# wjustin784/spMM

Hardware: AMD Instinct MI355X
Metric: CSR×CSR SpGEMM GFLOPS + peak HBM bytes, random N×N at stated density (higher is better)
Workload: dtype f64; 1 GPU; BASELINE config 4 (configs[3], ALG3 with its HBM cap): random CSR 65536x65536 density=0.005 float64 (spmm_amd.gen.random_csr on the device, seeds 42/43), ALG3, 1 chunk (cap not binding: the unchunked workspace is within chunk_fraction x P entries), chunk_fraction 0.2; N=65536, rows_per_rank=65536, alg=3, n_chunks=1, alg3_cap=not binding, nnzB=21465793, nnzA=21479711, nnzC=3460266668, num_products=7035505794, parallelism=single GPU

## Files before the change

spmm_amd/csrc/spgemm.hip:

```cpp
#include <hip/hip_runtime.h>
#include <hip/hip_ext.h>

#include <algorithm>
#include <atomic>
#include <cmath>
#include <cstdint>
#include <cstdio>
#include <cstdlib>
#include <cstring>
#include <limits>
#include <new>
#include <vector>

#include "spgemm.h"
#include "spgemm_kernels.hpp"
#include "spgemm_tile.hpp"
#include "spgemm_tile_dn.hpp"
#include "spgemm_spmv.hpp"
#include "spgemm_row.hpp"
#include "spgemm_spmm.hpp"
#include "spgemm_transpose.hpp"
#include "spgemm_geam.hpp"
#include "spgemm_canon.hpp"
#include "spgemm_extract.hpp"
#include "spgemm_dense.hpp"

using namespace spg;

constexpr int PINNED_WORDS = MIRROR_GEN_WORD + 1;

struct spg_handle_s {
    int device = 0;
    int cus = 256;
    hipStream_t stream = nullptr;
    int last_hip = 0;
    int64_t* pinned = nullptr;
    int64_t mirror_gen = 0;
    int32_t* spill_ctr = nullptr;
    bool spill_ctr_dirty = false;
    uint64_t lb_spin = SCAN_SPIN;
    bool lds_ordered = true;
    bool lds_ordered32 = true;
    void* scratch = nullptr;
    size_t scratch_bytes = 0;
    bool timing = false;
    struct Pending { int phase; hipEvent_t a, b; };
    std::vector<Pending> pending;
    std::vector<hipEvent_t> pool;
    double ms[SPG_NUM_PHASES] = {};
    int64_t launches[SPG_NUM_PHASES] = {};
    bool q_valid = false;
    spg_csr_t q_A{}, q_B{};
    spg_alg_t q_alg = SPG_ALG2;
    float q_cf = 0.f;
    int64_t q_P = -1, q_seg_len = 0;
    std::vector<int64_t> q_chunk_rows, q_chunk_nz;
};

struct spg_plan_s {
    spg_csr_t A{}, B{};
    spg_alg_t alg = SPG_ALG2;
    float cf = 0.2f;
    char* ws = nullptr;
    size_t ws_bytes = 0;
    int64_t* scalars = nullptr;
    int64_t* row_cnt = nullptr;
    uint32_t* seg = nullptr;
// ... 13 lines not shown
    bool lean = true;
    bool lean32 = true;
    int tws = 10;
    int G = 1;
    int rgs = 0;
    int twss = 10;
    bool sym_seg = false;
    bool sym_flags = false;
    bool counts_ready = false;
    unsigned long long* lb = nullptr;
    void* ext = nullptr;
    bool alg1_fused = false;
    bool fused_failed = false;
    bool scaled_in_place = false;
    int64_t sym_spills = -1;
    int64_t nspc = 0;
    int64_t* cspill = nullptr;
    std::vector<int64_t> chunk_spills;
    int64_t cap = 0;
    uint2* tidx = nullptr;
    int32_t* tptr = nullptr;
    bool packed = false;
    bool placed = false;
    uint2* pseg = nullptr;
    int32_t* segblk = nullptr;
    uint32_t* sidx = nullptr;
    void* brec = nullptr;
    uint16_t* bj16 = nullptr;
    bool brec_built = false;
    bool brec_cols = false;
    uint32_t* bitmap = nullptr;
    int64_t* item_cnt = nullptr;
    bool tidx_built = false;
    unsigned list_grid = 16;
    int symbolic_runs = 0;
    std::vector<int64_t> chunk_rows;
    std::vector<int64_t> chunk_nz;
};

namespace {

inline size_t align_up(size_t x, size_t a = 256) { return (x + a - 1) / a * a; }

inline size_t vbytes(spg_dtype_t t) {
    return t == SPG_C_64F ? 16 : (t == SPG_R_64F || t == SPG_C_32F) ? 8 : 4;
}

inline size_t brec_bytes(spg_dtype_t t) {
    return t == SPG_R_64F ? 10 : t == SPG_R_32F ? 6 : 4 + vbytes(t);
}

template <typename F>
spg_status_t dispatch_value(spg_dtype_t t, F&& f) {
    switch (t) {
#ifndef SPG_ONLY_F64
        case SPG_R_32F: return f(float(0));
        case SPG_C_32F: return f(cplx<float>(0));
        case SPG_C_64F: return f(cplx<double>(0));
#endif
        case SPG_R_64F: return f(double(0));
        default: break;
    }
    return SPG_STATUS_NOT_SUPPORTED;
}

template <typename F>
// ... 187 lines not shown
    return e;
}

struct PhaseTimer {
    spg_handle_t h;
    int phase;
    hipEvent_t a = nullptr;
    PhaseTimer(spg_handle_t h_, int phase_) : h(h_), phase(phase_) {
        if (h->timing && (a = take_event(h))) (void)hipEventRecord(a, h->stream);
    }
    ~PhaseTimer() {
        if (!a) return;
        hipEvent_t b = take_event(h);
        if (!b) { h->pool.push_back(a); return; }
        (void)hipEventRecord(b, h->stream);
        h->pending.push_back({phase, a, b});
    }
};

struct KernelTimer {
    spg_handle_t h;
    int phase;
    hipEvent_t a = nullptr, b = nullptr;
    KernelTimer(spg_handle_t h_, int phase_) : h(h_), phase(phase_) {
        if (!h->timing || !(a = take_event(h))) return;
        if (!(b = take_event(h))) { h->pool.push_back(a); a = nullptr; }
    }
    ~KernelTimer() {
        if (a && b) h->pending.push_back({phase, a, b});
    }
};

template <typename K, typename... Args>
inline void timed_launch(spg_handle_t h, int phase, K kernel, dim3 grid, dim3 block, Args... args) {
    KernelTimer kt(h, phase);
    hipExtLaunchKernelGGL(kernel, grid, block, 0, h->stream, kt.a, kt.b, 0, args...);
}

spg_status_t check_csr(const spg_csr_t* M) {
    if (!M) return SPG_STATUS_INVALID_VALUE;
    if (M->rows < 0 || M->cols < 0 || M->nnz < 0) return SPG_STATUS_INVALID_VALUE;
    if (M->cols > 2147483647LL) return SPG_STATUS_NOT_SUPPORTED;
    if (M->indptr_type != SPG_INDEX_32I && M->indptr_type != SPG_INDEX_64I)
        return SPG_STATUS_INVALID_VALUE;
    if (M->value_type != SPG_R_32F && M->value_type != SPG_R_64F && M->value_type != SPG_C_32F &&
        M->value_type != SPG_C_64F)
        return SPG_STATUS_NOT_SUPPORTED;
    if (M->indptr_type == SPG_INDEX_32I && M->nnz > 2147483647LL) return SPG_STATUS_INVALID_VALUE;
    if (!M->indptr && M->rows >= 0) return SPG_STATUS_INVALID_VALUE;
    if (M->nnz > 0 && (!M->indices || !M->values)) return SPG_STATUS_INVALID_VALUE;
    return SPG_STATUS_SUCCESS;
}

spg_status_t ensure_scratch(spg_handle_t h, size_t bytes) {
    if (h->scratch_bytes >= bytes) return SPG_STATUS_SUCCESS;
    if (h->scratch) {
        SPG_HIP(h, hipStreamSynchronize(h->stream));
        SPG_HIP(h, hipFree(h->scratch));
        h->scratch = nullptr;
        h->scratch_bytes = 0;
    }
    SPG_HIP(h, hipMalloc(&h->scratch, bytes));
    h->scratch_bytes = bytes;
    return SPG_STATUS_SUCCESS;
}

template <typename OUT, typename IN = int64_t>
spg_status_t launch_scan(spg_handle_t h, int64_t n, const IN* in, OUT* out,
                         unsigned long long* status, int64_t* scal, bool zero_status,
                         int32_t* move_cnt = nullptr, int64_t* move_dst = nullptr,
                         int64_t* host_mirror = nullptr, int64_t mirror_gen = 0, int mirror_n = 0,
                         const int64_t* seed = nullptr) {
    const int64_t tiles = scan_tiles(n);
    if (zero_status) SPG_HIP(h, hipMemsetAsync(status, 0, status_bytes(n), h->stream));
    timed_launch(h, SPG_PHASE_SCAN, k_scan_lb<OUT, IN>, dim3((unsigned)tiles), dim3(BLOCK), n, in, out, status, scal,
                 move_cnt, move_dst, host_mirror, mirror_gen, mirror_n, seed, h->lb_spin);
    SPG_LAUNCHED(h);
    return SPG_STATUS_SUCCESS;
}

template <typename IP>
spg_status_t launch_products(spg_handle_t h, const spg_csr_t& A, const spg_csr_t& B,
                             int64_t* cnt, int64_t* pref, int64_t* scal,
                             unsigned long long* status, bool zero_status) {
    const int64_t rows = A.rows;
    if (rows > 0) {
        PhaseTimer pt(h, SPG_PHASE_PRODUCTS);
        hipLaunchKernelGGL(k_row_products<IP>, dim3((unsigned)grid_for(rows, WPB)), dim3(BLOCK), 0,
                           h->stream, rows, (const IP*)A.indptr, (const int32_t*)A.indices,
                           (const IP*)B.indptr, cnt);
        SPG_LAUNCHED(h);
    }
    return launch_scan<int64_t>(h, rows, cnt, pref, status, scal, zero_status);
}

spg_status_t products_prefix(spg_handle_t h, const spg_csr_t& A, const spg_csr_t& B,
                             int64_t* cnt, int64_t* pref, int64_t* scal,
                             unsigned long long* status, bool zero_status = true) {
    return dispatch_index(A.indptr_type, [&](auto ip) {
        return launch_products<decltype(ip)>(h, A, B, cnt, pref, scal, status, zero_status);
    });
}

spg_status_t read_scalars(spg_handle_t h, const int64_t* dev, int n, int64_t* out);

spg_status_t products_total(spg_handle_t h, const spg_csr_t& A, const spg_csr_t& B, int64_t* P) {
    spg_status_t st = ensure_scratch(h, 256);
    if (st) return st;
    unsigned long long* acc = (unsigned long long*)h->scratch;
    SPG_HIP(h, hipMemsetAsync(acc, 0, sizeof(unsigned long long), h->stream));
    if (A.nnz > 0) {
// ... 84 lines not shown
    return e && std::strcmp(e, "1") == 0;
}
inline int64_t tile_item_slots(const spg_plan_s& p) { return tile_dense(p) ? p.A.rows * p.G : tile_items(p); }
inline int64_t* tile_chunk_items(const spg_plan_s& p, int64_t c) {
    return tile_dense(p) ? p.item_cnt + tile_chunk_r0(p, c) * p.G : p.item_cnt;
}
inline int sym_tiles(const spg_plan_s& p) { const int R = 1 << (p.twss - p.tws); return (p.G + R - 1) / R; }
inline int64_t rec_groups(const spg_plan_s& p) { return ((int64_t)p.G + (1 << p.rgs) - 1) >> p.rgs; }
inline int64_t tiles_padded(const spg_plan_s& p) { return rec_groups(p) << p.rgs; }
inline int64_t group_words(const spg_plan_s& p) { return (p.B.rows << p.rgs) + 1; }
inline int64_t bt_entries(const spg_plan_s& p) { return p.use_tile ? rec_groups(p) * group_words(p) : 0; }
constexpr double F32_RUN_MIN = 48;
inline bool fp32_runs(const spg_plan_s& p) {
    if (!p.lean32 || p.A.value_type != SPG_R_32F || p.B.cols <= 0 || p.B.rows <= 0 || (1 << p.tws) > 1024) return false;
    const char* e = std::getenv("SPG_F32_RUNS");
    if (e && std::strcmp(e, "0") == 0) return false;
    const double seg = (double)p.B.nnz / (double)p.B.rows * (double)(1 << p.tws) / (double)p.B.cols;
    return seg >= F32_RUN_MIN;
}
inline bool packed_segments(const spg_plan_s& p) {
    if (!tile_dense(p)) return false;
    if (p.A.value_type == SPG_R_32F) return fp32_runs(p);
    return p.lean && (p.A.value_type == SPG_R_64F || p.A.value_type == SPG_C_64F);
}
constexpr double SEG_PLACE_MIN_PRODUCTS = 4.0e9;
inline bool placed_segments(const spg_plan_s& p) {
    if (!packed_segments(p) || p.B.rows <= 0 || p.B.cols <= 0) return false;
    const char* e = std::getenv("SPG_SEG_PLACE");
    if (e && (std::strcmp(e, "1") == 0 || std::strcmp(e, "0") == 0)) return e[0] == '1';
    const double avgB = (double)p.B.nnz / (double)p.B.rows;
    const double seg = avgB * (double)(1 << p.tws) / (double)p.B.cols;
    return seg * (double)brec_bytes(p.A.value_type) <= (double)SEG_PLACE_MAX &&
           (double)p.A.nnz * avgB >= SEG_PLACE_MIN_PRODUCTS;
}
inline int64_t seg_blocks(const spg_plan_s& p) { return p.placed ? (int64_t)p.G * grid_for(p.B.rows, SEG_BLK) : 0; }
inline size_t brec_span(const spg_plan_s& p) {
    const size_t rb = brec_bytes(p.A.value_type);
    if (!p.placed) return rb * (size_t)p.B.nnz;
    return align_up((size_t)seg_bound((uint64_t)p.B.nnz, (uint64_t)p.B.rows * (uint64_t)p.G, (uint32_t)rb), SEG_LINE);
}
constexpr int SP_RGS = 3;
inline int record_group_log2(const spg_plan_s& p) {
    if (!p.use_tile || tile_dense(p) || !p.lean) return 0;
    if (p.A.value_type != SPG_R_64F || p.tws != 13) return 0;
    const char* e = std::getenv("SPG_SP_RECORD_GROUP");
    if (e && std::strcmp(e, "1") == 0) return 0;
    return SP_RGS;
}

inline bool fused_alg1(const spg_plan_s& p) {
    return p.alg == SPG_ALG1 && p.use_short && !p.use_tile && p.A.rows <= (1LL << 24);
}
inline bool alg1_upper_bound(const spg_plan_s& p) { return p.alg == SPG_ALG1 && !p.use_tile && !fused_alg1(p); }

inline size_t status_words(const spg_plan_s& p) {
    return 2 * (size_t)(scan_tiles(p.A.rows) + 1) +
           (p.use_tile ? (size_t)scan_tiles(tile_items(p)) + 1 + (size_t)scan_tiles(bt_entries(p)) + 1 : 0) +
           (p.placed ? (size_t)scan_tiles(seg_blocks(p)) + 1 : 0) +
           (fused_alg1(p) ? (size_t)std::max<int64_t>(grid_for(p.A.rows, ShortSmall::WPB), row_groups(p.A.rows)) + 1 : 0);
}
inline unsigned long long* rowptr_scan_status(const spg_plan_s& p) { return p.scan_status + scan_tiles(p.A.rows) + 1; }
inline unsigned long long* item_scan_status(const spg_plan_s& p) {
    return p.scan_status + 2 * (scan_tiles(p.A.rows) + 1);
}
inline unsigned long long* bt_scan_status(const spg_plan_s& p) {
    return item_scan_status(p) + scan_tiles(tile_items(p)) + 1;
// ... 232 lines not shown
                                   (RowExt<IP>*)nullptr, RowScan<OFF>{});
            else
                hipLaunchKernelGGL((k_short<T, IP, OFF, MODE, ShortSmall>), dim3((unsigned)grid_for(n, ShortSmall::WPB)),
                                   dim3(ShortSmall::WPB * WAVE), 0, h->stream, r0, n, p.B.cols, Ap, Aj, Ax, Bp, Bj,
                                   Bx, off, cj, cx, alpha, p.row_cnt, l1, cnt, (const int32_t*)nullptr,
                                   (const int32_t*)nullptr, (unsigned long long*)nullptr, (OFF*)nullptr,
                                   (int64_t*)nullptr, (int64_t)0);
            SPG_LAUNCHED(h);
        }
        if (p.sym_spills == 0) return SPG_STATUS_SUCCESS;
        PhaseTimer ps(h, SPG_PHASE_SPILL);
        hipLaunchKernelGGL((k_numeric<T, IP, OFF, UB>), dim3(p.list_grid), dim3(BLOCK), 0, h->stream,
                           r0, n, p.B.cols, Ap, Aj, Ax, Bp, Bj, Bx, off, cj, cx, alpha, p.row_cnt,
                           p.seg, nz0, p.seg_len, (const int32_t*)l1, (const int32_t*)cnt);
    } else {
        PhaseTimer pt(h, SPG_PHASE_NUMERIC);
        hipLaunchKernelGGL((k_numeric<T, IP, OFF, UB>), dim3((unsigned)grid_for(n, WPB)), dim3(BLOCK), 0,
                           h->stream, r0, n, p.B.cols, Ap, Aj, Ax, Bp, Bj, Bx, off, cj, cx, alpha,
                           p.row_cnt, p.seg, nz0, p.seg_len, (const int32_t*)nullptr,
                           (const int32_t*)nullptr);
    }
    SPG_LAUNCHED(h);
    return SPG_STATUS_SUCCESS;
}

template <typename OUT>
spg_status_t run_scan(spg_handle_t h, spg_plan_s& p, void* out, int mirror_n = 0) {
    return launch_scan<OUT>(h, p.A.rows, (const int64_t*)p.row_cnt, (OUT*)out,
                            rowptr_scan_status(p), p.scalars, false, nullptr, nullptr,
                            mirror_n ? h->pinned : nullptr, mirror_n ? ++h->mirror_gen : 0, mirror_n);
}

template <typename IP>
spg_status_t tile_build_index(spg_handle_t h, spg_plan_s& p) {
    if (p.tidx_built) return SPG_STATUS_SUCCESS;
    const IP* Bp = (const IP*)p.B.indptr;
    const int32_t* Bj = (const int32_t*)p.B.indices;
    const int R = 1 << (p.twss - p.tws);
    {
        const int Gp = (int)tiles_padded(p);
        timed_launch(h, SPG_PHASE_LAYOUT, k_tile_index<IP>, dim3((unsigned)grid_for(p.B.rows, 4)), dim3(256), p.B.rows,
                     Bp, Bj, p.tws, Gp, p.tidx);
        SPG_LAUNCHED(h);
        const int64_t n2 = p.B.rows * Gp + rec_groups(p);
        timed_launch(h, SPG_PHASE_LAYOUT, k_bt_count,
                     dim3((unsigned)std::max<int64_t>(1, std::min<int64_t>(grid_for(n2, 256), 65536))), dim3(256),
                     p.B.rows, Gp, p.G, R, (const uint2*)p.tidx, p.tptr, p.sidx, p.rgs);
        SPG_LAUNCHED(h);
        timed_launch(h, SPG_PHASE_LAYOUT, k_bj16,
                     dim3((unsigned)std::max<int64_t>(1, std::min<int64_t>(grid_for(p.B.nnz, 256), 65536))), dim3(256),
                     p.B.nnz, Bj, p.bj16);
        SPG_LAUNCHED(h);
    }
    spg_status_t st = launch_scan<int32_t, int32_t>(h, bt_entries(p), p.tptr, p.tptr, bt_scan_status(p),
                                                    p.scalars + 2, false);
    if (st) return st;
    if (p.placed) {
        const int64_t nblk = seg_blocks(p);
        const dim3 grid((unsigned)std::max<int64_t>(1, grid_for(nblk, 256)));
        const uint32_t rb = (uint32_t)brec_bytes(p.A.value_type);
        timed_launch(h, SPG_PHASE_LAYOUT, k_seg_place<false>, grid, dim3(256), p.B.rows, p.G, rb,
                     (const int32_t*)p.tptr, p.segblk, p.pseg, (char*)p.brec);
        SPG_LAUNCHED(h);
        if ((st = launch_scan<int32_t, int32_t>(h, nblk, p.segblk, p.segblk, seg_scan_status(p), p.scalars + 6, false)))
            return st;
        timed_launch(h, SPG_PHASE_LAYOUT, k_seg_place<true>, grid, dim3(256), p.B.rows, p.G, rb,
                     (const int32_t*)p.tptr, p.segblk, p.pseg, (char*)p.brec);
        SPG_LAUNCHED(h);
    }
    p.tidx_built = true;
    return SPG_STATUS_SUCCESS;
}

template <typename IP>
spg_status_t tile_sym_chunk(spg_handle_t h, spg_plan_s& p, int64_t c) {
    const int64_t r0 = tile_chunk_r0(p, c), n = tile_chunk_r1(p, c) - r0;
    int64_t* items = tile_chunk_items(p, c);
    if (n > 0) {
        if (p.sym_flags) {
            constexpr int W = SYM_FLAG_W;
            KernelTimer kt(h, SPG_PHASE_SYMBOLIC);
            hipExtLaunchKernelGGL((k_tile_sym_flag<IP, W>), dim3(coop_grid(n * sym_tiles(p), W)), dim3(W * WAVE),
                                  (size_t)1 << p.twss, h->stream, kt.a, kt.b, 0, r0, n, p.tws, p.G, p.twss,
                                  (const IP*)p.A.indptr, (const int32_t*)p.A.indices, (const IP*)p.B.indptr,
                                  (const uint16_t*)p.bj16, (const uint32_t*)p.sidx, items);
        } else if (p.sym_seg) {
            timed_launch(h, SPG_PHASE_SYMBOLIC, k_tile_sym_seg<IP>, dim3(tile_grid(n * sym_tiles(p), SEG_WPB)),
                         dim3(SEG_WPB * WAVE), r0, n, p.tws, p.G, p.twss, (const IP*)p.A.indptr,
                         (const int32_t*)p.A.indices, (const IP*)p.B.indptr, (const uint16_t*)p.bj16,
                         (const uint32_t*)p.sidx, tile_dense(p) ? (uint32_t*)nullptr : p.bitmap, items,
                         sym_full(p) ? p.B.cols : (int64_t)0);
        } else {
            timed_launch(h, SPG_PHASE_SYMBOLIC, k_tile_sym8c<IP, SYM8_CW>,
                         dim3(coop_grid(n * sym_tiles(p), SYM8_CW)), dim3(SYM8_CW * WAVE),
                         r0, n, p.tws, p.G, p.twss, (const IP*)p.A.indptr, (const int32_t*)p.A.indices,
                         (const IP*)p.B.indptr, (const uint16_t*)p.bj16, (const uint32_t*)p.sidx,
                         tile_dense(p) ? (uint32_t*)nullptr : p.bitmap, items);
        }
        SPG_LAUNCHED(h);
    }
    const int64_t nch = tile_chunks(p);
    int64_t* scal = c == nch - 1 ? p.scalars : p.scalars + 12 + 2 * (c & 1);
    const int64_t* seed = c == 0 ? nullptr : p.scalars + 12 + 2 * ((c - 1) & 1);
    return launch_scan<int64_t>(h, n * p.G, (const int64_t*)items, items, item_scan_status(p), scal,
                                true, nullptr, nullptr, nullptr, 0, 0, seed);
}

template <typename OUT>
spg_status_t tile_rowptr_chunk(spg_handle_t h, spg_plan_s& p, int64_t c, void* cp) {
    const int64_t r0 = tile_chunk_r0(p, c), n = tile_chunk_r1(p, c) - r0;
    timed_launch(h, SPG_PHASE_SCAN, k_items_to_rowptr<OUT>, dim3((unsigned)grid_for(n + 1, 256)), dim3(256), n, p.G,
                 (const int64_t*)tile_chunk_items(p, c), (OUT*)cp + r0);
    SPG_LAUNCHED(h);
    return SPG_STATUS_SUCCESS;
}

template <typename IP, typename OUT>
spg_status_t tile_symbolic(spg_handle_t h, spg_plan_s& p, void* cp) {
    spg_status_t st;
    if ((st = tile_build_index<IP>(h, p))) return st;
    const int64_t nch = tile_chunks(p);
    if ((nch == 1 || tile_dense(p)) && p.counts_ready) {
        for (int64_t c = 0; c < nch; ++c)
            if ((st = tile_rowptr_chunk<OUT>(h, p, c, cp))) return st;
        return SPG_STATUS_SUCCESS;
    }
    for (int64_t c = 0; c < nch; ++c) {
        if ((st = tile_sym_chunk<IP>(h, p, c))) return st;
        if ((st = tile_rowptr_chunk<OUT>(h, p, c, cp))) return st;
    }
    return SPG_STATUS_SUCCESS;
}

template <typename T, typename IP>
spg_status_t tile_numeric(spg_handle_t h, spg_plan_s& p, int32_t* cj, T* cx, T alpha, int64_t g0 = 0,
                          int64_t g1 = -1, const T* tm = nullptr) {
    if (g1 < 0) g1 = p.G;
    const IP* Ap = (const IP*)p.A.indptr;
    const IP* Bp = (const IP*)p.B.indptr;
    const int32_t* Aj = (const int32_t*)p.A.indices;
    const int32_t* Bj = (const int32_t*)p.B.indices;
    const T* Ax = (const T*)p.A.values;
    const T* Bx = (const T*)p.B.values;
    if (tm) {
        if (!p.brec_cols) {
            timed_launch(h, SPG_PHASE_LAYOUT, k_bt_pack<T, IP, 1>, dim3((unsigned)grid_for(p.B.rows, 4)), dim3(256),
                         p.B.rows, Bp, Bj, Bx, p.tws, (const int32_t*)p.tptr, (uint32_t*)p.brec, p.B.nnz, (T*)nullptr,
                         p.rgs, p.pseg, seg_end(p), seg_pairs(p), p.G);
            SPG_LAUNCHED(h);
            p.brec_cols = true;
        }
        p.brec_built = false;
        const int32_t* tp = (const int32_t*)p.tptr;
        const int64_t W = group_words(p);
        const int64_t q0 = g0 >> p.rgs, q1 = (g1 + (1 << p.rgs) - 1) >> p.rgs;
        const int64_t est = std::max<int64_t>(1, p.B.nnz * (q1 - q0) / std::max<int64_t>(rec_groups(p), 1));
        if (p.placed)
            timed_launch(h, SPG_PHASE_LAYOUT, k_bt_fill_pk<T>,
                         dim3((unsigned)std::max<int64_t>(1, std::min<int64_t>(grid_for((q1 - q0) * grid_for(p.B.rows, WAVE), 4), 16384))),
                         dim3(256), p.B.rows, q0, q1, tp, (const uint2*)p.pseg, tm, (uint32_t*)p.brec);
        else
            timed_launch(h, SPG_PHASE_LAYOUT, k_bt_fill<T>,
                         dim3((unsigned)std::max<int64_t>(1, std::min<int64_t>(grid_for(est, 256), 16384))), dim3(256),
                         tp + q0 * W, tp + (q1 - 1) * W + (W - 1), tm, (uint32_t*)p.brec);
        SPG_LAUNCHED(h);
    } else if (!p.brec_built) {
        timed_launch(h, SPG_PHASE_LAYOUT, k_bt_pack<T, IP>, dim3((unsigned)grid_for(p.B.rows, 4)), dim3(256), p.B.rows,
                     Bp, Bj, Bx, p.tws, (const int32_t*)p.tptr, (uint32_t*)p.brec, p.B.nnz, (T*)nullptr, p.rgs,
                     p.pseg, seg_end(p), seg_pairs(p), p.G);
        SPG_LAUNCHED(h);
        p.brec_built = true;
        p.brec_cols = true;
    }
    auto sent = [&](int r) {
        return (uint32_t)(((uint64_t)(p.packed ? 0 : p.B.nnz) + (uint64_t)r * SENT_N) * (uint64_t)rec_bytes<T>());
    };
    const int64_t nch = tile_chunks(p);
    for (int64_t c = 0; c < nch; ++c) {
        spg_status_t st;
        if (nch > 1 && !tile_dense(p) && (st = tile_sym_chunk<IP>(h, p, c))) return st;
        const int64_t r0 = tile_chunk_r0(p, c), n = tile_chunk_r1(p, c) - r0;
        if (n <= 0) continue;
        uint32_t it_lo = (uint32_t)(g0 * n), it_hi = (uint32_t)(g1 * n);
        int64_t nit = (g1 - g0) * n;
        KernelTimer kt(h, SPG_PHASE_NUMERIC);
        const bool dense = tile_dense(p);
        auto launch = [&](auto dn) {
            constexpr bool DN = decltype(dn)::value;
            constexpr int WPBN = tile_num_wpb<DN>();
            hipExtLaunchKernelGGL((k_tile<T, IP, DN>), dim3(tile_grid(nit, WPBN)), dim3(WPBN * WAVE), 0,
                                  h->stream, kt.a, kt.b, 0, r0, n, p.tws, p.G, Ap, Aj, Ax, p.B.rows,
                                  (const uint32_t*)p.brec, (const int32_t*)p.tptr,
                                  dense ? (const uint32_t*)nullptr : (const uint32_t*)p.bitmap,
                                  (const int64_t*)tile_chunk_items(p, c), cj, cx, alpha, it_lo, it_hi, p.rgs);
        };
        if constexpr (std::is_same<T, float>::value) {
            if (dense && p.packed) {
                hipExtLaunchKernelGGL((k_tile_dn<T, IP, 1024>), dim3(tile_grid(nit, DN_WPB)), dim3(DN_WPB * WAVE),
                                      0, h->stream, kt.a, kt.b, 0, r0, n, p.tws, p.G, Ap, Aj, Ax, p.B.rows,
                                      (const uint32_t*)p.brec, (const uint2*)p.pseg, (const int32_t*)seg_end(p),
                                      (const int64_t*)tile_chunk_items(p, c), cj, cx, alpha,
                                      sent(sentinel_region(1024)), it_lo, it_hi);
                SPG_LAUNCHED(h);
                continue;
            }
// ... 231 lines not shown
spg_status_t symbolic_rows(spg_handle_t h, spg_plan_s& p, void* cp, spg_index_t ct, int64_t* nnzC);

spg_status_t symbolic_alg1_short(spg_handle_t h, spg_plan_s& p, void* cp, spg_index_t ct, int64_t* nnzC) {
    spg_status_t st;
    ++p.symbolic_runs;
    if (p.counts_ready) {
        SPG_HIP(h, hipMemsetAsync(rowptr_scan_status(p), 0, status_bytes(p.A.rows), h->stream));
        if ((st = dispatch_index(ct, [&](auto out) { return run_scan<decltype(out)>(h, p, cp); }))) return st;
        int64_t tot;
        if ((st = read_scalars(h, p.scalars, 1, &tot))) return st;
        if (past_int32(ct, tot)) return SPG_STATUS_OVERFLOW;
        return symbolic_done(p, cp, ct, tot, nnzC);
    }
    st = dispatch_value(p.A.value_type, [&](auto tag) {
        return dispatch_index(p.A.indptr_type, ct, [&](auto ip, auto out) {
            return alg1_short_launch<decltype(tag), decltype(ip), decltype(out)>(h, p, cp);
        });
    });
    if (st) return st;
    int64_t sc[11];
    if ((st = read_scalars(h, p.scalars, 11, sc))) return st;
    if (sc[LB_FAIL] || sc[LB_CAPX]) {
        p.fused_failed = true;
        p.symbolic_runs = 0;
        return symbolic_rows(h, p, cp, ct, nnzC);
    }
    p.counts_ready = true;
    p.alg1_fused = true;
    if (past_int32(ct, sc[LB_TOTAL])) return SPG_STATUS_OVERFLOW;
    return symbolic_done(p, cp, ct, sc[LB_TOTAL], nnzC);
}

spg_status_t symbolic_tiles(spg_handle_t h, spg_plan_s& p, void* cp, spg_index_t ct, int64_t* nnzC) {
    spg_status_t st = dispatch_index(p.A.indptr_type, ct, [&](auto ip, auto out) {
        return tile_symbolic<decltype(ip), decltype(out)>(h, p, cp);
    });
    if (st) return st;
    int64_t tot;
    if ((st = read_scalars(h, p.scalars, 1, &tot))) return st;
    p.counts_ready = true;
    if (past_int32(ct, tot)) return SPG_STATUS_OVERFLOW;
    return symbolic_done(p, cp, ct, tot, nnzC);
}

spg_status_t symbolic_rows(spg_handle_t h, spg_plan_s& p, void* cp, spg_index_t ct, int64_t* nnzC) {
    spg_status_t st;
    if (p.symbolic_runs++ > 0) {
        SPG_HIP(h, hipMemsetAsync(rowptr_scan_status(p), 0, status_bytes(p.A.rows), h->stream));
    }
    const bool counted = !p.counts_ready;
    if (counted) {
        if (alg1_upper_bound(p)) {
            st = dispatch_value(p.A.value_type, [&](auto tag) {
                using T = decltype(tag);
                return dispatch_index(p.A.indptr_type, [&](auto ip) {
                    return run_numeric_rows<T, decltype(ip), int64_t, true>(h, p, 0, p.A.rows, 0, p.ub, p.tj,
                                                                            (T*)p.tx, (T)1);
                });
            });
        } else {
            st = dispatch_index(p.A.indptr_type, [&](auto ip) { return symbolic_typed<decltype(ip)>(h, p); });
        }
        if (st) return st;
    }
    const bool chunks = p.nspc > 0 && counted;
    const int nread = chunks ? 16 + p.nspc : 5;
    if ((st = dispatch_index(ct, [&](auto out) { return run_scan<decltype(out)>(h, p, cp, nread); }))) return st;
    std::vector<int64_t> all((size_t)nread);
    if ((st = wait_mirror(h))) return st;
    for (int i = 0; i < nread; ++i) all[(size_t)i] = ((volatile int64_t*)h->pinned)[i];
    if (chunks) {
        p.chunk_spills.assign(all.begin() + 16, all.end());
// ... 730 lines not shown
        case SPG_STATUS_HIP_ERROR: return "SPG_STATUS_HIP_ERROR";
    }
    return "SPG_STATUS_UNKNOWN";
}

spg_status_t spg_create(spg_handle_t* handle, int hip_device) {
    if (!handle) return SPG_STATUS_INVALID_VALUE;
    *handle = nullptr;
    int ndev = 0;
    if (hipGetDeviceCount(&ndev) != hipSuccess || ndev <= 0) return SPG_STATUS_NOT_INITIALIZED;
    int dev = hip_device;
    if (dev < 0) {
        if (hipGetDevice(&dev) != hipSuccess) return SPG_STATUS_NOT_INITIALIZED;
    }
    if (dev >= ndev) return SPG_STATUS_INVALID_VALUE;
    hipDeviceProp_t prop;
    if (hipGetDeviceProperties(&prop, dev) != hipSuccess) return SPG_STATUS_NOT_INITIALIZED;
    if (std::strncmp(prop.gcnArchName, "gfx950", 6) != 0) return SPG_STATUS_ARCH_MISMATCH;
    spg_handle_s* h = new (std::nothrow) spg_handle_s();
    if (!h) return SPG_STATUS_ALLOC_FAILED;
    h->device = dev;
    h->cus = prop.multiProcessorCount > 0 ? prop.multiProcessorCount : 256;
    if (const char* e = std::getenv("SPG_LB_SPIN_TICKS")) h->lb_spin = std::strtoull(e, nullptr, 10);
    DeviceGuard dg_(dev);
    hipError_t e = dg_.err;
    if (e == hipSuccess) e = lds_order_check(&h->lds_ordered, &h->lds_ordered32);
    if (const char* o = std::getenv("SPG_LDS_ORDERED"))
        if (std::strcmp(o, "0") == 0) h->lds_ordered = h->lds_ordered32 = false;
    if (e == hipSuccess)
        e = hipHostMalloc((void**)&h->pinned, PINNED_WORDS * sizeof(int64_t), hipHostMallocCoherent | hipHostMallocMapped);
    if (e == hipSuccess) std::memset(h->pinned, 0, PINNED_WORDS * sizeof(int64_t));
    if (e == hipSuccess) e = hipMalloc((void**)&h->spill_ctr, 256);
    if (e == hipSuccess) e = hipMemset(h->spill_ctr, 0, 256);
    if (e != hipSuccess) {
        delete h;
        return e == hipErrorOutOfMemory ? SPG_STATUS_ALLOC_FAILED : SPG_STATUS_HIP_ERROR;
    }
    *handle = h;
    return SPG_STATUS_SUCCESS;
}

spg_status_t spg_destroy(spg_handle_t h) {
    if (!h) return SPG_STATUS_NOT_INITIALIZED;
    (void)hipStreamSynchronize(h->stream);
    if (h->scratch) (void)hipFree(h->scratch);
    if (h->pinned) (void)hipHostFree(h->pinned);
    if (h->spill_ctr) (void)hipFree(h->spill_ctr);
    for (auto& q : h->pending) { (void)hipEventDestroy(q.a); (void)hipEventDestroy(q.b); }
    for (hipEvent_t e : h->pool) (void)hipEventDestroy(e);
    delete h;
    return SPG_STATUS_SUCCESS;
}

spg_status_t spg_set_stream(spg_handle_t h, void* stream) {
    if (!h) return SPG_STATUS_NOT_INITIALIZED;
    if ((hipStream_t)stream != h->stream) SPG_HIP(h, hipStreamSynchronize(h->stream));
    h->stream = (hipStream_t)stream;
    return SPG_STATUS_SUCCESS;
}

int spg_last_hip_error(spg_handle_t h) { return h ? h->last_hip : 0; }

spg_status_t spg_plan(spg_handle_t h, const spg_csr_t* A, const spg_csr_t* B, spg_alg_t alg,
                      float chunk_fraction, size_t* workspace_bytes, void* workspace,
                      spg_plan_t* plan) {
    if (!h) return SPG_STATUS_NOT_INITIALIZED;
    if (!workspace_bytes) return SPG_STATUS_INVALID_VALUE;
    spg_status_t st;
    if ((st = check_csr(A)) || (st = check_csr(B))) return st;
    if (A->cols != B->rows) return SPG_STATUS_INVALID_VALUE;
    if (A->value_type != B->value_type) return SPG_STATUS_INVALID_VALUE;
    if (A->indptr_type != B->indptr_type) return SPG_STATUS_INVALID_VALUE;
    if (alg != SPG_ALG_DEFAULT && alg != SPG_ALG1 && alg != SPG_ALG2 && alg != SPG_ALG3)
        return SPG_STATUS_INVALID_VALUE;
    if (alg == SPG_ALG3 && !(chunk_fraction > 0.0f && chunk_fraction <= 1.0f))
        return SPG_STATUS_INVALID_VALUE;
    if (workspace && !plan) return SPG_STATUS_INVALID_VALUE;
    DeviceGuard dg_(h->device);
    SPG_HIP(h, dg_.err);

    spg_plan_s tmp;
    tmp.A = *A;
    tmp.B = *B;
    tmp.alg = alg == SPG_ALG_DEFAULT ? SPG_ALG2 : alg;
    tmp.cf = chunk_fraction;
    tmp.seg_len = A->nnz;
    tmp.use_short = want_short(*A, *B);
    tmp.use_row = row_kernel_enabled();
    tmp.lean = h->lds_ordered;
    tmp.lean32 = h->lds_ordered32;
    tmp.use_tile = !tmp.use_short && want_tile(*A, *B, tmp.tws, tmp.G, tmp.lean);
    if (tmp.use_tile) {
        tmp.twss = sym_tile_log2(*B, tmp.tws, &tmp.sym_seg);
        tmp.rgs = record_group_log2(tmp);
        tmp.packed = packed_segments(tmp);
        tmp.placed = placed_segments(tmp);
        tmp.sym_flags = want_sym_flags(tmp);
    }
    tmp.list_grid = (unsigned)std::max<int64_t>(1, std::min<int64_t>(256, grid_for(A->rows, 64)));
    const bool same_as_query = h->q_valid && h->q_alg == tmp.alg && h->q_cf == chunk_fraction &&
                               std::memcmp(&h->q_A, A, sizeof(spg_csr_t)) == 0 &&
                               std::memcmp(&h->q_B, B, sizeof(spg_csr_t)) == 0;
    if (fused_alg1(tmp)) {
        const double avgB = B->rows > 0 ? (double)B->nnz / (double)B->rows : 0.0;
        const double est = 1.15 * (double)A->nnz * avgB + 4096.0;
        const double full = (double)A->rows * (double)B->cols;
        tmp.cap = (int64_t)std::min(est, full);
    } else if (alg1_upper_bound(tmp)) {
        if (workspace && same_as_query) {
            tmp.P = h->q_P;
        } else if ((st = products_total(h, *A, *B, &tmp.P))) {
            return st;
        }
    } else if (tmp.alg == SPG_ALG3) {
        if (workspace && same_as_query) {
            tmp.P = h->q_P;
            tmp.chunk_rows = h->q_chunk_rows;
            tmp.chunk_nz = h->q_chunk_nz;
            tmp.seg_len = h->q_seg_len;
        } else {
            spg_plan_s whole = tmp;
            whole.chunk_rows.assign({0, A->rows});
            whole.chunk_nz.assign({0, A->nnz});
            whole.seg_len = tmp.use_tile ? 1 : A->nnz;
            const char* ae = std::getenv("SPG_ALG3_CHUNK_ALWAYS");
            const bool always = ae && std::strcmp(ae, "1") == 0;
            if ((st = products_total(h, *A, *B, &tmp.P))) return st;
            const double cap = (double)chunk_fraction * (double)std::max<int64_t>(tmp.P, 0) *
                               (double)(sizeof(int32_t) + vbytes(A->value_type));
            if (always || (double)make_layout(whole).total > cap) {
// ... 572 lines not shown
    if (!p || !info || capacity < 0 || (capacity > 0 && !chunk_rows)) return SPG_STATUS_INVALID_VALUE;
    info->path = p->use_tile ? 2 : (p->use_short ? 1 : 0);
    info->tile_width = p->use_tile ? (1 << p->tws) : 0;
    info->tiles_per_row = p->use_tile ? p->G : 0;
    info->record_group = p->use_tile ? (1 << p->rgs) : 0;
    info->dense_tiles = tile_dense(*p) ? 1 : 0;
    const bool chunked = p->alg == SPG_ALG3 && p->chunk_rows.size() > 1;
    info->n_chunks = chunked ? (int64_t)p->chunk_rows.size() - 1 : 1;
    info->lds_ordered = p->use_tile && p->lean && (p->A.value_type == SPG_R_64F || p->A.value_type == SPG_C_64F) ? 1 : 0;
    if (tile_dense(*p) && fp32_runs(*p)) info->lds_ordered = 1;
    for (int64_t i = 0; i < std::min<int64_t>(capacity, info->n_chunks + 1); ++i)
        chunk_rows[i] = chunked ? p->chunk_rows[(size_t)i] : (i == 0 ? 0 : p->A.rows);
    return SPG_STATUS_SUCCESS;
}

spg_status_t spg_plan_destroy(spg_plan_t p) {
    if (!p) return SPG_STATUS_INVALID_VALUE;
    delete p;
    return SPG_STATUS_SUCCESS;
}

spg_status_t spg_spgemm_ws(spg_handle_t h, const spg_csr_t* A, const spg_csr_t* B, spg_alg_t alg,
                           float chunk_fraction, const void* alpha, void* workspace, size_t workspace_bytes,
                           void* C_indptr, spg_index_t C_indptr_type, int64_t* nnzC, void** C_indices,
                           void** C_values, size_t* peak_bytes, spg_plan_t* plan_out) {
    if (!h) return SPG_STATUS_NOT_INITIALIZED;
    if (!alpha || !nnzC || !C_indices || !C_values || !peak_bytes || !plan_out) return SPG_STATUS_INVALID_VALUE;
    *plan_out = nullptr;
    *C_indices = *C_values = nullptr;
    spg_plan_t p = nullptr;
    size_t wsb = workspace_bytes;
    spg_status_t st = spg_plan(h, A, B, alg, chunk_fraction, &wsb, workspace, &p);
    if (st) return st;
    if ((st = spg_symbolic(h, p, C_indptr, C_indptr_type, nnzC))) {
        spg_plan_destroy(p);
        return st;
    }
    const size_t ipc = C_indptr_type == SPG_INDEX_32I ? 4 : 8;
    if (p->alg1_fused && *nnzC > 0) {
        spg_csr_t C{p->A.rows, p->B.cols, *nnzC, C_indptr, p->tj, p->tx, C_indptr_type, p->A.value_type};
        st = spg_numeric(h, p, alpha, &C);
        if (!st) {
            *C_indices = p->tj;
            *C_values = p->tx;
            *peak_bytes = p->ws_bytes + ipc * (size_t)(p->A.rows + 1);
        }
        spg_plan_destroy(p);
        return st;
    }
    *peak_bytes = p->ws_bytes + ipc * (size_t)(p->A.rows + 1) +
                  (size_t)*nnzC * (sizeof(int32_t) + vbytes(p->A.value_type));
    *plan_out = p;
    return SPG_STATUS_SUCCESS;
}

spg_status_t spg_set_timing(spg_handle_t h, int enable) {
    if (!h) return SPG_STATUS_NOT_INITIALIZED;
    SPG_HIP(h, hipStreamSynchronize(h->stream));
    for (auto& q : h->pending) { h->pool.push_back(q.a); h->pool.push_back(q.b); }
    h->pending.clear();
    for (int i = 0; i < SPG_NUM_PHASES; ++i) { h->ms[i] = 0.0; h->launches[i] = 0; }
    h->timing = enable != 0;
    return SPG_STATUS_SUCCESS;
}

spg_status_t spg_get_timing(spg_handle_t h, spg_timing_t* t) {
// ... 18 lines not shown
```

spmm_amd/cusparse.py:

```python
from __future__ import annotations

import ctypes
from dataclasses import dataclass

import numpy as np
import torch

from . import _fastpath, _lib
from ._lib import SpgCsr, SpgError, check
from .sparse import csr_matrix

_VT = {torch.float32: _lib.SPG_R_32F, torch.float64: _lib.SPG_R_64F,
       torch.complex64: _lib.SPG_C_32F, torch.complex128: _lib.SPG_C_64F}
_ALPHA_CT = {torch.float32: (ctypes.c_float, 1), torch.float64: (ctypes.c_double, 1),
             torch.complex64: (ctypes.c_float, 2), torch.complex128: (ctypes.c_double, 2)}
_IT = {torch.int32: _lib.SPG_INDEX_32I, torch.int64: _lib.SPG_INDEX_64I}
_ALG = {1: _lib.SPG_ALG1, 2: _lib.SPG_ALG2, 3: _lib.SPG_ALG3}


@dataclass
class SpgemmStats:
    alg: int = 0
    workspace_bytes: int = 0
    peak_bytes: int = 0
# ... 132 lines not shown
    if before_numeric is not None and algo == _lib.SPG_ALG1:
        before_numeric()
        before_numeric = None
    if by_tiles is not None and algo == _lib.SPG_ALG1:
        if by_tiles(None) is not None:
            raise RuntimeError("by_tiles must complete B's values when geom is None")
        by_tiles = None
    if by_tiles is not None:
        return _spgemm_by_tiles(h, a, b, alpha, algo, cf, by_tiles, verbose, values_first)
    if fp is not None:
        al = complex(alpha)
        st, data, indices, indptr, wsb, peak = fp.spgemm(
            h.ptr.value, m, a.shape[1], n, a.indptr, a.indices, a.data, b.indptr, b.indices, b.data,
            int(algo), cf, al.real, al.imag)
        check(st, "spg_spgemm_ws")
        if verbose:
            print("USING ALG", alg, "workspace GB =", wsb / (1024 ** 3))
        last_stats.alg, last_stats.workspace_bytes = int(algo), int(wsb)
        last_stats.peak_bytes, last_stats.nnz = int(peak), int(indices.numel())
        return csr_matrix._from_parts(data, indices, indptr, (m, n), canonical=True)
    lib = h.lib
    va, vb = _csr_view(a), _csr_view(b)
    ws_bytes = ctypes.c_size_t(0)
    check(lib.spg_plan(h.ptr, ctypes.byref(va), ctypes.byref(vb), algo, cf,
                       ctypes.byref(ws_bytes), None, None), "spg_plan")
    if verbose:
        print("USING ALG", alg, "workspace GB =", ws_bytes.value / (1024 ** 3))
    ws = torch.empty(max(ws_bytes.value, 1), dtype=torch.uint8, device=dev)
    ct, nparts = _ALPHA_CT[a.data.dtype]
    al = (ct * 2)(complex(alpha).real, complex(alpha).imag) if nparts == 2 else ct(float(alpha))
    nnz, peak = ctypes.c_int64(0), ctypes.c_size_t(0)
    pj, px, plan = ctypes.c_void_p(), ctypes.c_void_p(), ctypes.c_void_p()
    wide = a.nnz * (b.nnz / max(b.shape[0], 1)) >= 2 ** 31
    for it in ((torch.int64,) if wide else (torch.int32, torch.int64)):
        indptr = torch.empty(m + 1, dtype=it, device=dev)
        st = lib.spg_spgemm_ws(h.ptr, ctypes.byref(va), ctypes.byref(vb), algo, cf, ctypes.byref(al),
                               ctypes.c_void_p(ws.data_ptr()), ws_bytes.value,
                               ctypes.c_void_p(indptr.data_ptr()), _IT[it], ctypes.byref(nnz),
                               ctypes.byref(pj), ctypes.byref(px), ctypes.byref(peak), ctypes.byref(plan))
        if st != _lib.STATUS_OVERFLOW:
            break
    check(st, "spg_spgemm_ws")
    nnzc = int(nnz.value)
    if pj.value:
        base = ws.data_ptr()
        oj, ox = pj.value - base, px.value - base
        indices = ws[oj:oj + 4 * nnzc].view(torch.int32)
        data = ws[ox:ox + a.data.element_size() * nnzc].view(a.data.dtype)
    else:
        try:
            indices = torch.empty(nnzc, dtype=torch.int32, device=dev)
            data = torch.empty(nnzc, dtype=a.data.dtype, device=dev)
            vc = SpgCsr(m, n, nnzc, indptr.data_ptr(), indices.data_ptr() if nnzc else 0,
                        data.data_ptr() if nnzc else 0, _IT[indptr.dtype], _VT[data.dtype])
            if before_numeric is not None:
                before_numeric()
            check(lib.spg_numeric(h.ptr, plan, ctypes.byref(al), ctypes.byref(vc)), "spg_numeric")
        finally:
            lib.spg_plan_destroy(plan)
    if wide and nnzc < 2 ** 31:
        indptr = indptr.to(torch.int32)
    last_stats.alg, last_stats.workspace_bytes = int(algo), int(ws_bytes.value)
    last_stats.peak_bytes, last_stats.nnz = int(peak.value), nnzc
    return csr_matrix._from_parts(data, indices, indptr, (m, n), canonical=True)


def _alpha_of(dtype, alpha):
    ct, nparts = _ALPHA_CT[dtype]
    return (ct * 2)(complex(alpha).real, complex(alpha).imag) if nparts == 2 else ct(float(alpha))


def _spgemm_by_tiles(h, a, b, alpha, algo, cf, by_tiles, verbose, values_first=True):
    lib = h.lib
    m, n = a.shape[0], b.shape[1]
    dev = a.device
# ... 682 lines not shown
```

Before: 695.3 GFLOPS.

## Overlap tile layout scan and record packing with symbolic phase on side stream

Splits the B tile-index build into a head (index, count, bj16) on the main stream and a tail (scan, segment placement, and optionally early record packing) run on a new side stream forked by event. The symbolic row-pointer chunks run concurrently on the main stream, and the main stream waits on a join event afterwards. When the chunks are mirrored, the symbolic total is read through a pinned host mirror instead of a device readback. The Python path also changes to call plan/symbolic separately when before_numeric is set. The cost is extra stream/event management, and any ordering mistake between the streams would be a hazard.

Measured after the change: 675.7 GFLOPS. 0.972x the previous value.

```diff
diff --git a/spmm_amd/csrc/spgemm.hip b/spmm_amd/csrc/spgemm.hip
--- a/spmm_amd/csrc/spgemm.hip
+++ b/spmm_amd/csrc/spgemm.hip
@@ -33,6 +33,8 @@
     int device = 0;
     int cus = 256;
     hipStream_t stream = nullptr;
+    hipStream_t side = nullptr;
+    hipEvent_t ev_fork = nullptr, ev_join = nullptr;
     int last_hip = 0;
     int64_t* pinned = nullptr;
     int64_t mirror_gen = 0;
@@ -112,6 +114,8 @@
     uint32_t* bitmap = nullptr;
     int64_t* item_cnt = nullptr;
     bool tidx_built = false;
+    bool overlap = true;
+    bool pack_early = false;
     unsigned list_grid = 16;
     int symbolic_runs = 0;
     std::vector<int64_t> chunk_rows;
@@ -365,9 +369,14 @@
 };
 
 template <typename K, typename... Args>
+inline void timed_launch_on(spg_handle_t h, hipStream_t stream, int phase, K kernel, dim3 grid, dim3 block,
+                            Args... args) {
+    KernelTimer kt(h, phase);
+    hipExtLaunchKernelGGL(kernel, grid, block, 0, stream, kt.a, kt.b, 0, args...);
+}
+template <typename K, typename... Args>
 inline void timed_launch(spg_handle_t h, int phase, K kernel, dim3 grid, dim3 block, Args... args) {
-    KernelTimer kt(h, phase);
-    hipExtLaunchKernelGGL(kernel, grid, block, 0, h->stream, kt.a, kt.b, 0, args...);
+    timed_launch_on(h, h->stream, phase, kernel, grid, block, args...);
 }
 
 spg_status_t check_csr(const spg_csr_t* M) {
@@ -399,17 +408,26 @@
 }
 
 template <typename OUT, typename IN = int64_t>
+spg_status_t launch_scan_on(spg_handle_t h, hipStream_t stream, int64_t n, const IN* in, OUT* out,
+                            unsigned long long* status, int64_t* scal, bool zero_status,
+                            int32_t* move_cnt = nullptr, int64_t* move_dst = nullptr,
+                            int64_t* host_mirror = nullptr, int64_t mirror_gen = 0, int mirror_n = 0,
+                            const int64_t* seed = nullptr) {
+    const int64_t tiles = scan_tiles(n);
+    if (zero_status) SPG_HIP(h, hipMemsetAsync(status, 0, status_bytes(n), stream));
+    timed_launch_on(h, stream, SPG_PHASE_SCAN, k_scan_lb<OUT, IN>, dim3((unsigned)tiles), dim3(BLOCK), n, in, out,
+                    status, scal, move_cnt, move_dst, host_mirror, mirror_gen, mirror_n, seed, h->lb_spin);
+    SPG_LAUNCHED(h);
+    return SPG_STATUS_SUCCESS;
+}
+template <typename OUT, typename IN = int64_t>
 spg_status_t launch_scan(spg_handle_t h, int64_t n, const IN* in, OUT* out,
                          unsigned long long* status, int64_t* scal, bool zero_status,
                          int32_t* move_cnt = nullptr, int64_t* move_dst = nullptr,
                          int64_t* host_mirror = nullptr, int64_t mirror_gen = 0, int mirror_n = 0,
                          const int64_t* seed = nullptr) {
-    const int64_t tiles = scan_tiles(n);
-    if (zero_status) SPG_HIP(h, hipMemsetAsync(status, 0, status_bytes(n), h->stream));
-    timed_launch(h, SPG_PHASE_SCAN, k_scan_lb<OUT, IN>, dim3((unsigned)tiles), dim3(BLOCK), n, in, out, status, scal,
-                 move_cnt, move_dst, host_mirror, mirror_gen, mirror_n, seed, h->lb_spin);
-    SPG_LAUNCHED(h);
-    return SPG_STATUS_SUCCESS;
+    return launch_scan_on<OUT, IN>(h, h->stream, n, in, out, status, scal, zero_status, move_cnt, move_dst,
+                                   host_mirror, mirror_gen, mirror_n, seed);
 }
 
 template <typename IP>
@@ -560,6 +578,10 @@
     const double seg = avgB * (double)(1 << p.tws) / (double)p.B.cols;
     return seg * (double)brec_bytes(p.A.value_type) <= (double)SEG_PLACE_MAX &&
            (double)p.A.nnz * avgB >= SEG_PLACE_MIN_PRODUCTS;
+}
+inline bool layout_overlap() {
+    const char* e = std::getenv("SPG_LAYOUT_OVERLAP");
+    return !(e && std::strcmp(e, "0") == 0);
 }
 inline int64_t seg_blocks(const spg_plan_s& p) { return p.placed ? (int64_t)p.G * grid_for(p.B.rows, SEG_BLK) : 0; }
 inline size_t brec_span(const spg_plan_s& p) {
@@ -858,48 +880,70 @@
 }
 
 template <typename IP>
-spg_status_t tile_build_index(spg_handle_t h, spg_plan_s& p) {
-    if (p.tidx_built) return SPG_STATUS_SUCCESS;
+spg_status_t tile_index_head(spg_handle_t h, spg_plan_s& p) {
     const IP* Bp = (const IP*)p.B.indptr;
     const int32_t* Bj = (const int32_t*)p.B.indices;
     const int R = 1 << (p.twss - p.tws);
-    {
-        const int Gp = (int)tiles_padded(p);
-        timed_launch(h, SPG_PHASE_LAYOUT, k_tile_index<IP>, dim3((unsigned)grid_for(p.B.rows, 4)), dim3(256), p.B.rows,
-                     Bp, Bj, p.tws, Gp, p.tidx);
-        SPG_LAUNCHED(h);
-        const int64_t n2 = p.B.rows * Gp + rec_groups(p);
-        timed_launch(h, SPG_PHASE_LAYOUT, k_bt_count,
-                     dim3((unsigned)std::max<int64_t>(1, std::min<int64_t>(grid_for(n2, 256), 65536))), dim3(256),
-                     p.B.rows, Gp, p.G, R, (const uint2*)p.tidx, p.tptr, p.sidx, p.rgs);
-        SPG_LAUNCHED(h);
-        timed_launch(h, SPG_PHASE_LAYOUT, k_bj16,
-                     dim3((unsigned)std::max<int64_t>(1, std::min<int64_t>(grid_for(p.B.nnz, 256), 65536))), dim3(256),
-                     p.B.nnz, Bj, p.bj16);
-        SPG_LAUNCHED(h);
-    }
-    spg_status_t st = launch_scan<int32_t, int32_t>(h, bt_entries(p), p.tptr, p.tptr, bt_scan_status(p),
-                                                    p.scalars + 2, false);
+    const int Gp = (int)tiles_padded(p);
+    timed_launch(h, SPG_PHASE_LAYOUT, k_tile_index<IP>, dim3((unsigned)grid_for(p.B.rows, 4)), dim3(256), p.B.rows,
+                 Bp, Bj, p.tws, Gp, p.tidx);
+    SPG_LAUNCHED(h);
+    const int64_t n2 = p.B.rows * Gp + rec_groups(p);
+    timed_launch(h, SPG_PHASE_LAYOUT, k_bt_count,
+                 dim3((unsigned)std::max<int64_t>(1, std::min<int64_t>(grid_for(n2, 256), 65536))), dim3(256),
+                 p.B.rows, Gp, p.G, R, (const uint2*)p.tidx, p.tptr, p.sidx, p.rgs);
+    SPG_LAUNCHED(h);
+    timed_launch(h, SPG_PHASE_LAYOUT, k_bj16,
+                 dim3((unsigned)std::max<int64_t>(1, std::min<int64_t>(grid_for(p.B.nnz, 256), 65536))), dim3(256),
+                 p.B.nnz, Bj, p.bj16);
+    SPG_LAUNCHED(h);
+    return SPG_STATUS_SUCCESS;
+}
+
+inline spg_status_t tile_index_tail(spg_handle_t h, spg_plan_s& p, hipStream_t stream) {
+    spg_status_t st = launch_scan_on<int32_t, int32_t>(h, stream, bt_entries(p), p.tptr, p.tptr, bt_scan_status(p),
+                                                       p.scalars + 2, false);
     if (st) return st;
     if (p.placed) {
         const int64_t nblk = seg_blocks(p);
         const dim3 grid((unsigned)std::max<int64_t>(1, grid_for(nblk, 256)));
         const uint32_t rb = (uint32_t)brec_bytes(p.A.value_type);
-        timed_launch(h, SPG_PHASE_LAYOUT, k_seg_place<false>, grid, dim3(256), p.B.rows, p.G, rb,
-                     (const int32_t*)p.tptr, p.segblk, p.pseg, (char*)p.brec);
+        timed_launch_on(h, stream, SPG_PHASE_LAYOUT, k_seg_place<false>, grid, dim3(256), p.B.rows, p.G, rb,
+                        (const int32_t*)p.tptr, p.segblk, p.pseg, (char*)p.brec);
         SPG_LAUNCHED(h);
-        if ((st = launch_scan<int32_t, int32_t>(h, nblk, p.segblk, p.segblk, seg_scan_status(p), p.scalars + 6, false)))
+        if ((st = launch_scan_on<int32_t, int32_t>(h, stream, nblk, p.segblk, p.segblk, seg_scan_status(p),
+                                                   p.scalars + 6, false)))
             return st;
-        timed_launch(h, SPG_PHASE_LAYOUT, k_seg_place<true>, grid, dim3(256), p.B.rows, p.G, rb,
-                     (const int32_t*)p.tptr, p.segblk, p.pseg, (char*)p.brec);
+        timed_launch_on(h, stream, SPG_PHASE_LAYOUT, k_seg_place<true>, grid, dim3(256), p.B.rows, p.G, rb,
+                        (const int32_t*)p.tptr, p.segblk, p.pseg, (char*)p.brec);
         SPG_LAUNCHED(h);
     }
+    return SPG_STATUS_SUCCESS;
+}
+
+template <typename IP>
+spg_status_t tile_build_index(spg_handle_t h, spg_plan_s& p) {
+    if (p.tidx_built) return SPG_STATUS_SUCCESS;
+    spg_status_t st;
+    if ((st = tile_index_head<IP>(h, p)) || (st = tile_index_tail(h, p, h->stream))) return st;
     p.tidx_built = true;
     return SPG_STATUS_SUCCESS;
 }
 
+template <typename T, typename IP>
+spg_status_t tile_pack_records(spg_handle_t h, spg_plan_s& p, hipStream_t stream) {
+    timed_launch_on(h, stream, SPG_PHASE_LAYOUT, k_bt_pack<T, IP>, dim3((unsigned)grid_for(p.B.rows, 4)), dim3(256),
+                    p.B.rows, (const IP*)p.B.indptr, (const int32_t*)p.B.indices, (const T*)p.B.values, p.tws,
+                    (const int32_t*)p.tptr, (uint32_t*)p.brec, p.B.nnz, (T*)nullptr, p.rgs, p.pseg, seg_end(p),
+                    seg_pairs(p), p.G);
+    SPG_LAUNCHED(h);
+    p.brec_built = true;
+    p.brec_cols = true;
+    return SPG_STATUS_SUCCESS;
+}
+
 template <typename IP>
-spg_status_t tile_sym_chunk(spg_handle_t h, spg_plan_s& p, int64_t c) {
+spg_status_t tile_sym_chunk(spg_handle_t h, spg_plan_s& p, int64_t c, bool mirror = false) {
     const int64_t r0 = tile_chunk_r0(p, c), n = tile_chunk_r1(p, c) - r0;
     int64_t* items = tile_chunk_items(p, c);
     if (n > 0) {
@@ -928,8 +972,10 @@
     const int64_t nch = tile_chunks(p);
     int64_t* scal = c == nch - 1 ? p.scalars : p.scalars + 12 + 2 * (c & 1);
     const int64_t* seed = c == 0 ? nullptr : p.scalars + 12 + 2 * ((c - 1) & 1);
+    const bool mir = mirror && c == nch - 1;
     return launch_scan<int64_t>(h, n * p.G, (const int64_t*)items, items, item_scan_status(p), scal,
-                                true, nullptr, nullptr, nullptr, 0, 0, seed);
+                                true, nullptr, nullptr, mir ? h->pinned : nullptr, mir ? ++h->mirror_gen : 0,
+                                mir ? 1 : 0, seed);
 }
 
 template <typename OUT>
@@ -942,20 +988,47 @@
 }
 
 template <typename IP, typename OUT>
-spg_status_t tile_symbolic(spg_handle_t h, spg_plan_s& p, void* cp) {
+spg_status_t tile_symbolic_chunks(spg_handle_t h, spg_plan_s& p, void* cp, bool& mirrored) {
     spg_status_t st;
-    if ((st = tile_build_index<IP>(h, p))) return st;
     const int64_t nch = tile_chunks(p);
-    if ((nch == 1 || tile_dense(p)) && p.counts_ready) {
-        for (int64_t c = 0; c < nch; ++c)
-            if ((st = tile_rowptr_chunk<OUT>(h, p, c, cp))) return st;
-        return SPG_STATUS_SUCCESS;
-    }
+    mirrored = !((nch == 1 || tile_dense(p)) && p.counts_ready);
     for (int64_t c = 0; c < nch; ++c) {
-        if ((st = tile_sym_chunk<IP>(h, p, c))) return st;
+        if (mirrored && (st = tile_sym_chunk<IP>(h, p, c, true))) return st;
         if ((st = tile_rowptr_chunk<OUT>(h, p, c, cp))) return st;
     }
     return SPG_STATUS_SUCCESS;
+}
+
+template <typename IP>
+spg_status_t tile_layout_aside(spg_handle_t h, spg_plan_s& p) {
+    SPG_HIP(h, hipStreamWaitEvent(h->side, h->ev_fork, 0));
+    spg_status_t st = tile_index_tail(h, p, h->side);
+    if (st) return st;
+    if (p.pack_early) {
+        st = dispatch_value(p.A.value_type, [&](auto tag) { return tile_pack_records<decltype(tag), IP>(h, p, h->side); });
+        if (st) return st;
+    }
+    SPG_HIP(h, hipEventRecord(h->ev_join, h->side));
+    return SPG_STATUS_SUCCESS;
+}
+
+template <typename IP, typename OUT>
+spg_status_t tile_symbolic(spg_handle_t h, spg_plan_s& p, void* cp, bool& mirrored) {
+    spg_status_t st;
+    if (p.tidx_built || !p.overlap) {
+        if ((st = tile_build_index<IP>(h, p))) return st;
+        return tile_symbolic_chunks<IP, OUT>(h, p, cp, mirrored);
+    }
+    if ((st = tile_index_head<IP>(h, p))) return st;
+    SPG_HIP(h, hipEventRecord(h->ev_fork, h->stream));
+    if (!(st = tile_layout_aside<IP>(h, p))) {
+        p.tidx_built = true;
+        st = tile_symbolic_chunks<IP, OUT>(h, p, cp, mirrored);
+    }
+    const hipError_t join = st ? hipSuccess : hipStreamWaitEvent(h->stream, h->ev_join, 0);
+    if (!st && join == hipSuccess) return SPG_STATUS_SUCCESS;
+    (void)hipStreamSynchronize(h->side);
+    return st ? st : hip_fail(h, join);
 }
 
 template <typename T, typename IP>
@@ -991,12 +1064,8 @@
                          tp + q0 * W, tp + (q1 - 1) * W + (W - 1), tm, (uint32_t*)p.brec);
         SPG_LAUNCHED(h);
     } else if (!p.brec_built) {
-        timed_launch(h, SPG_PHASE_LAYOUT, k_bt_pack<T, IP>, dim3((unsigned)grid_for(p.B.rows, 4)), dim3(256), p.B.rows,
-                     Bp, Bj, Bx, p.tws, (const int32_t*)p.tptr, (uint32_t*)p.brec, p.B.nnz, (T*)nullptr, p.rgs,
-                     p.pseg, seg_end(p), seg_pairs(p), p.G);
-        SPG_LAUNCHED(h);
-        p.brec_built = true;
-        p.brec_cols = true;
+        spg_status_t st = tile_pack_records<T, IP>(h, p, h->stream);
+        if (st) return st;
     }
     auto sent = [&](int r) {
         return (uint32_t)(((uint64_t)(p.packed ? 0 : p.B.nnz) + (uint64_t)r * SENT_N) * (uint64_t)rec_bytes<T>());
@@ -1294,12 +1363,18 @@
 }
 
 spg_status_t symbolic_tiles(spg_handle_t h, spg_plan_s& p, void* cp, spg_index_t ct, int64_t* nnzC) {
+    bool mirrored = false;
     spg_status_t st = dispatch_index(p.A.indptr_type, ct, [&](auto ip, auto out) {
-        return tile_symbolic<decltype(ip), decltype(out)>(h, p, cp);
+        return tile_symbolic<decltype(ip), decltype(out)>(h, p, cp, mirrored);
     });
     if (st) return st;
     int64_t tot;
-    if ((st = read_scalars(h, p.scalars, 1, &tot))) return st;
+    if (mirrored) {
+        if ((st = wait_mirror(h))) return st;
+        tot = ((volatile int64_t*)h->pinned)[0];
+    } else if ((st = read_scalars(h, p.scalars, 1, &tot))) {
+        return st;
+    }
     p.counts_ready = true;
     if (past_int32(ct, tot)) return SPG_STATUS_OVERFLOW;
     return symbolic_done(p, cp, ct, tot, nnzC);
@@ -2096,7 +2171,13 @@
     if (e == hipSuccess) std::memset(h->pinned, 0, PINNED_WORDS * sizeof(int64_t));
     if (e == hipSuccess) e = hipMalloc((void**)&h->spill_ctr, 256);
     if (e == hipSuccess) e = hipMemset(h->spill_ctr, 0, 256);
+    if (e == hipSuccess) e = hipStreamCreateWithFlags(&h->side, hipStreamNonBlocking);
+    if (e == hipSuccess) e = hipEventCreateWithFlags(&h->ev_fork, hipEventDisableTiming);
+    if (e == hipSuccess) e = hipEventCreateWithFlags(&h->ev_join, hipEventDisableTiming);
     if (e != hipSuccess) {
+        if (h->ev_join) (void)hipEventDestroy(h->ev_join);
+        if (h->ev_fork) (void)hipEventDestroy(h->ev_fork);
+        if (h->side) (void)hipStreamDestroy(h->side);
         delete h;
         return e == hipErrorOutOfMemory ? SPG_STATUS_ALLOC_FAILED : SPG_STATUS_HIP_ERROR;
     }
@@ -2107,6 +2188,10 @@
 spg_status_t spg_destroy(spg_handle_t h) {
     if (!h) return SPG_STATUS_NOT_INITIALIZED;
     (void)hipStreamSynchronize(h->stream);
+    (void)hipStreamSynchronize(h->side);
+    (void)hipEventDestroy(h->ev_join);
+    (void)hipEventDestroy(h->ev_fork);
+    (void)hipStreamDestroy(h->side);
     if (h->scratch) (void)hipFree(h->scratch);
     if (h->pinned) (void)hipHostFree(h->pinned);
     if (h->spill_ctr) (void)hipFree(h->spill_ctr);
@@ -2160,6 +2245,7 @@
         tmp.packed = packed_segments(tmp);
         tmp.placed = placed_segments(tmp);
         tmp.sym_flags = want_sym_flags(tmp);
+        tmp.overlap = layout_overlap();
     }
     tmp.list_grid = (unsigned)std::max<int64_t>(1, std::min<int64_t>(256, grid_for(A->rows, 64)));
     const bool same_as_query = h->q_valid && h->q_alg == tmp.alg && h->q_cf == chunk_fraction &&
@@ -2798,6 +2884,7 @@
     size_t wsb = workspace_bytes;
     spg_status_t st = spg_plan(h, A, B, alg, chunk_fraction, &wsb, workspace, &p);
     if (st) return st;
+    p->pack_early = p->overlap;
     if ((st = spg_symbolic(h, p, C_indptr, C_indptr_type, nnzC))) {
         spg_plan_destroy(p);
         return st;
diff --git a/spmm_amd/cusparse.py b/spmm_amd/cusparse.py
--- a/spmm_amd/cusparse.py
+++ b/spmm_amd/cusparse.py
@@ -188,15 +188,26 @@
     nnz, peak = ctypes.c_int64(0), ctypes.c_size_t(0)
     pj, px, plan = ctypes.c_void_p(), ctypes.c_void_p(), ctypes.c_void_p()
     wide = a.nnz * (b.nnz / max(b.shape[0], 1)) >= 2 ** 31
+    if before_numeric is not None:
+        check(lib.spg_plan(h.ptr, ctypes.byref(va), ctypes.byref(vb), algo, cf, ctypes.byref(ws_bytes),
+                           ctypes.c_void_p(ws.data_ptr()), ctypes.byref(plan)), "spg_plan")
     for it in ((torch.int64,) if wide else (torch.int32, torch.int64)):
         indptr = torch.empty(m + 1, dtype=it, device=dev)
-        st = lib.spg_spgemm_ws(h.ptr, ctypes.byref(va), ctypes.byref(vb), algo, cf, ctypes.byref(al),
-                               ctypes.c_void_p(ws.data_ptr()), ws_bytes.value,
-                               ctypes.c_void_p(indptr.data_ptr()), _IT[it], ctypes.byref(nnz),
-                               ctypes.byref(pj), ctypes.byref(px), ctypes.byref(peak), ctypes.byref(plan))
+        if before_numeric is not None:
+            st = lib.spg_symbolic(h.ptr, plan, ctypes.c_void_p(indptr.data_ptr()), _IT[it], ctypes.byref(nnz))
+        else:
+            st = lib.spg_spgemm_ws(h.ptr, ctypes.byref(va), ctypes.byref(vb), algo, cf, ctypes.byref(al),
+                                   ctypes.c_void_p(ws.data_ptr()), ws_bytes.value,
+                                   ctypes.c_void_p(indptr.data_ptr()), _IT[it], ctypes.byref(nnz),
+                                   ctypes.byref(pj), ctypes.byref(px), ctypes.byref(peak), ctypes.byref(plan))
         if st != _lib.STATUS_OVERFLOW:
             break
-    check(st, "spg_spgemm_ws")
+    if before_numeric is not None:
+        if st == 0:
+            st = lib.spg_peak_bytes(plan, ctypes.byref(peak))
+        if st != 0:
+            lib.spg_plan_destroy(plan)
+    check(st, "spg_symbolic" if before_numeric is not None else "spg_spgemm_ws")
     nnzc = int(nnz.value)
     if pj.value:
         base = ws.data_ptr()
```
